# TravisWheelerLab/sufr

Hardware: AMD Instinct MI355X
Metric: suffixes sorted/sec (SA+LCP) (higher is better)
Workload: dtype u8 text / u32 indices / u64 packed keys; 1 GPU; syn_human 3.1 Gb stand-in for GRCh38, --dna --ignore-softmask -n 256 (BASELINE configs[3]); text_len=3100000001, num_suffixes=1500223556, parallelism=prefix-bucket shards x1, bits_per_char=3, radix_passes=5, digit_bits=15, levels=7, deep_records=58357696, placement_trials=3

## Files before the change

### profiles/micro/level2_pattern.hip

```cpp
#include <hip/hip_runtime.h>
#include <stdint.h>
#include <stdio.h>
#include <stdlib.h>
#include <vector>
#define CK(x) do { hipError_t e_ = (x); if (e_ != hipSuccess) { fprintf(stderr, "%s: %s\n", #x, hipGetErrorString(e_)); exit(1); } } while (0)
struct Rec12 { uint32_t a, b, c; };
struct Rec8 { uint32_t a, b; };

template <typename OUT>
__global__ void __launch_bounds__(512)
k_level2(const Rec12* __restrict__ in, OUT* __restrict__ out, uint32_t* __restrict__ cursor, uint32_t NB, uint32_t r, uint32_t SEG,
         uint32_t nseg)
{
    extern __shared__ uint32_t s_base[];
    const uint32_t g = blockIdx.x & 7u, w = blockIdx.x >> 3, R = gridDim.x >> 3;
    const uint32_t tile = NB * r, tps = SEG / tile;
    for (uint32_t seg = g; seg < nseg; seg += 8) {
        for (uint32_t t = w; t < tps; t += R) {
            __syncthreads();
            for (uint32_t d = threadIdx.x; d < NB; d += 512)
                s_base[d] = seg * SEG + d * (SEG / NB) + atomicAdd(&cursor[(size_t)seg * NB + d], r);
            __syncthreads();
            const Rec12* src = in + (size_t)seg * SEG + (size_t)t * tile;
            for (uint32_t j = threadIdx.x; j < tile; j += 512) {
                const Rec12 v = src[j];
                const uint32_t d = j / r, o = j - d * r;
                if constexpr (sizeof(OUT) == 12) out[(size_t)s_base[d] + o] = OUT{v.a, v.b, v.c};
                else out[(size_t)s_base[d] + o] = OUT{v.a ^ v.b, v.c};
            }
        }
    }
}

int main(int argc, char** argv)
{
    const uint32_t NB = argc > 1 ? (uint32_t)atoi(argv[1]) : 1400u;
    const uint32_t nseg = 1364;
    hipEvent_t e0, e1; CK(hipEventCreate(&e0)); CK(hipEventCreate(&e1));
    for (uint32_t r : {1u, 2u, 3u, 6u}) {
        const uint32_t tile = NB * r;
        const uint32_t SEG = (1100000u / tile) * tile;
        const uint64_t records = (uint64_t)SEG * nseg;
        Rec12* in; void* out; uint32_t* cursor;
        CK(hipMalloc(&in, records * 12)); CK(hipMalloc(&out, records * 12)); CK(hipMalloc(&cursor, (size_t)nseg * NB * 4));
        CK(hipMemset(in, 1, records * 12));
        for (int sz : {12, 8}) {
            float best = 1e9f;
            for (int rep = 0; rep < 3; rep++) {
                CK(hipMemset(cursor, 0, (size_t)nseg * NB * 4));
                CK(hipEventRecord(e0));
                if (sz == 12) hipLaunchKernelGGL(k_level2<Rec12>, dim3(1024), dim3(512), (size_t)NB * 4, 0, in, (Rec12*)out, cursor, NB, r, SEG, nseg);
                else hipLaunchKernelGGL(k_level2<Rec8>, dim3(1024), dim3(512), (size_t)NB * 4, 0, in, (Rec8*)out, cursor, NB, r, SEG, nseg);
                CK(hipEventRecord(e1)); CK(hipEventSynchronize(e1));
                float ms; CK(hipEventElapsedTime(&ms, e0, e1)); best = ms < best ? ms : best;
            }
            printf("sub-buckets %5u  run %u rec  out %2d B/rec : %7.2f ms  (%.3g records, %.1f GB read, %.1f GB written)\n", NB, r, sz, best,
                   (double)records, records * 12.0 / 1e9, records * (double)sz / 1e9);
        }
        CK(hipFree(in)); CK(hipFree(out)); CK(hipFree(cursor));
    }
    return 0;
}
```

### sufr_amd/csrc/sufr_launch.inc

```

#include <math.h>
#include <stdio.h>
#include <stdlib.h>
#include <string.h>

#include <chrono>
#include <memory>
#include <string>
#include <thread>
#include <vector>

#include "../../include/sufr_hip.h"

namespace sufr {

#define HIP_TRY(call)                                                                        \
    do {                                                                                     \
        hipError_t e__ = (call);                                                             \
        if (e__ != hipSuccess) {                                                             \
            set_error(std::string(#call) + ": " + hipGetErrorString(e__));                   \
            return SUFR_HIP_E_HIP;                                                           \
        }                                                                                    \
    } while (0)

// ... 23 lines not shown
    std::string err;
    uint64_t resident_text_len = 0;
    uint32_t stitch_weight = 0;
    uint64_t stitch_cap = 0;
    DevBuf stitchoffs;
    StitchOrder stitch_order() const { StitchOrder so; so.offs = stitch_weight ? (const uint32_t*)stitchoffs.p : nullptr; so.weight = stitch_weight; so.cap = stitch_cap; return so; }
    bool debug = false;

    DevBuf text, bytehist, lut, table, bintot, binbase, scalars;
    DevBuf keyA, keyB, idxA, idxB;
    DevBuf recA, recB;
    DevBuf rankbuf, dposbuf, deferbuf, unresbuf, posbitsbuf, dblf[7], dblg[6];
    DevBuf headsA, headsB, sizes, starts, partials;
    DevBuf tilefirst, runends, tileany, nexttile, nextblk, depthA, depthB, period, remapbuf, flagsbuf, packedbuf, wmaskbuf, wcntbuf, recoff, runoff, wlflag, wlhead, wloff, candbuf, keepbuf, plancnt, fixbuf;
    DevBuf rg_misc, rg_blk, rg_blkoff, rg_rs, rg_rl, rg_E, rg_L, rg_V, rg_tab[2], rg_off[2], rg_long[2], rg_tmax[2], rg_hist, rg_depth;
    DevBuf cumbuf, dmapbuf, identbuf[16], grouptab, gcur, leafcnt, leafoff, leafbase, leafcur, bigflag, bigoff;
    DevBuf rawtab, presbuf, rawtot, valsbuf, startbuf;
    DevBuf exc_pos, exc_byte, exc_sorted, exc_sa, exc_lcp, exc_bits, exc_blk, exc_off, exc_list, exc_list2, exc_pmin, exc_roff;
    std::unique_ptr<Pipeline> helper;
    bool overlap_chains = true;
    bool mql_fast_ok = true;
    bool exc_disable = false;
    bool no_exceptions = false;
    std::vector<uint32_t> rawtot_host, valshost;
    uint16_t h_lut[256];
    uint32_t h_seg0[2];
    DevBuf segst[2], segsz[2], tunits, upre, tdesc, wunits, wpre, wdesc, wslow;
    std::vector<uint8_t> dmaphost, identhost[16];
    std::vector<uint16_t> remaphost;
    std::vector<uint32_t> cumhost;
    int segcur = 0;
// ... 28 lines not shown
    uint32_t wide_shard_index = 0, wide_num_shards = 1;
    uint64_t wide_text_len = 0;
    uint64_t wide_orphans = 0;
    std::vector<uint32_t> opt_mask_offsets;
    hipEvent_t ev[16];
    bool have_events = false;

    static constexpr int LEAF_E = 8;
    int leaf_nt = 512;
    uint32_t LEAF_CAP = 4096;
    uint32_t LEAF_BIG = 4096;
    bool leaf_dna3 = false;
    uint32_t leaf_bmax = 256;
    int leaf_t1 = 12;
    int ms_e = 8;
    static constexpr int ms_nt = 512;

    void set_error(const std::string& s) { err = s; }

    static constexpr size_t PIN_CAP = (size_t)512 << 10;
    uint8_t* pin = nullptr;
    size_t pin_used = 0;
    struct PinItem { void* dst; size_t off, bytes; };
    std::vector<PinItem> pin_items;
    hipError_t d2h_at(void* dst, const void* src, size_t bytes)
    {
        if (!pin || pin_used + bytes > PIN_CAP) { copies_queued = true; return hipMemcpyAsync(dst, src, bytes, hipMemcpyDeviceToHost, stream); }
        const hipError_t e = hipMemcpyAsync(pin + pin_used, src, bytes, hipMemcpyDeviceToHost, stream);
        if (e == hipSuccess) { pin_items.push_back({dst, pin_used, bytes}); pin_used += (bytes + 63) & ~(size_t)63; copies_queued = true; }
        return e;
// ... 140 lines not shown
        if (const char* e = getenv("SUFR_PROBE_LEAF_BIG")) if (atoi(e) >= 64) LEAF_BIG = (uint32_t)atoi(e);
        if (LEAF_BIG > LEAF_CAP) LEAF_BIG = LEAF_CAP;
        if (const char* e = getenv("SUFR_PROBE_FINISH_OPTS")) finish_opts = (uint32_t)atoi(e) << 29;
        if (const char* e = getenv("SUFR_PROBE_DBL_SHARE")) dbl_min_share = (uint32_t)atoi(e);
        if (const char* e = getenv("SUFR_PROBE_P2MIN")) p2min_knob = atoi(e);
        key_carry = !getenv("SUFR_PROBE_NO_KEY_CARRY");
        run_groups = !getenv("SUFR_PROBE_NO_RUN_GROUPS");
        mask_lcp_from_keys = !getenv("SUFR_PROBE_MASK_LCP_TEXT");
        if (const char* e = getenv("SUFR_PROBE_MASK_DIGIT_BITS")) { int v = atoi(e); if (v >= 4 && v <= 12) mask_digit_bits = v; }
        if (const char* e = getenv("SUFR_PROBE_GROUP_SORT")) group_sort = atoi(e) != 0;
        if (const char* e = getenv("SUFR_PROBE_GIANT")) if (atoi(e) >= (int)GS_CAP) gs_giant_knob = (uint32_t)atoi(e);
        if (const char* e = getenv("SUFR_PROBE_KEY_CHARS")) key_chars_knob = atoi(e);
        if (const char* e = getenv("SUFR_PROBE_BMAX")) if (atoi(e) >= 1) leaf_bmax = (uint32_t)atoi(e);
        if (const char* e = getenv("SUFR_PROBE_LEAF_ABL")) leaf_bmax |= (uint32_t)atoi(e) << 24;
        if (const char* e = getenv("SUFR_PROBE_MS_E")) if (atoi(e) == 4 || atoi(e) == 6 || atoi(e) == 8) ms_e = atoi(e);
        if (const char* e = getenv("SUFR_PROBE_T1")) if (atoi(e) >= 11 && atoi(e) <= 13) leaf_t1 = atoi(e);
        if (leaf_nt == 512 && leaf_t1 == 13) leaf_t1 = 12;
        if (leaf_nt == 1024 && leaf_t1 == 11) leaf_t1 = 12;
#endif
        if (text_wgs > 16384u) text_wgs = 16384u;
        if (pairs_wgs > 16384u) pairs_wgs = 16384u;
    }

    void release(DevBuf& b) { if (b.p) (void)hipFree(b.p); b.p = nullptr; b.cap = 0; }

    void destroy()
    {
        if (helper) { helper->destroy(); helper.reset(); }
        (void)hipSetDevice(device);
        DevBuf* all[] = {&text, &bytehist, &lut, &table, &bintot, &binbase, &scalars, &keyA, &keyB, &idxA,
                         &idxB, &recA, &recB, &headsA, &headsB, &sizes, &starts, &partials, &sa32, &lcp32,
                         &tilefirst, &runends, &tileany, &nexttile, &nextblk, &depthA, &depthB, &period, &remapbuf, &flagsbuf, &packedbuf, &wmaskbuf, &wcntbuf, &recoff, &runoff, &wlflag, &wlhead, &wloff, &candbuf, &keepbuf, &plancnt, &fixbuf,
                         &rg_misc, &rg_blk, &rg_blkoff, &rg_rs, &rg_rl, &rg_E, &rg_L, &rg_V, &rg_tab[0], &rg_tab[1], &rg_off[0], &rg_off[1], &rg_long[0], &rg_long[1], &rg_tmax[0], &rg_tmax[1], &rg_hist, &rg_depth,
                         &exc_pos, &exc_byte, &exc_sorted, &exc_sa, &exc_lcp, &exc_bits, &exc_blk, &exc_off, &exc_list, &exc_list2, &exc_pmin, &exc_roff,
                         &cumbuf, &dmapbuf, &rawtab, &presbuf, &rawtot, &valsbuf, &startbuf, &grouptab, &gcur, &leafcnt, &leafoff, &leafbase, &leafcur, &bigflag, &bigoff,
                         &segst[0], &segst[1], &segsz[0], &segsz[1], &tunits, &upre, &tdesc, &wunits, &wpre, &wdesc, &wslow,
                         &optA, &optB, &optC, &optD, &optE, &stitchoffs, &wideoffs,
                         &gs_leafbase, &gs_pst, &gs_psz, &gs_wcnt, &gs_wpre, &gs_wdesc, &gs_flag, &gs_off, &gs_big, &gs_lg, &gs_lsz, &gs_loff};
        for (auto& b : identbuf) release(b);
        for (auto& b : dblf) release(b);
        for (auto& b : dblg) release(b);
        release(rankbuf); release(dposbuf); release(deferbuf); release(unresbuf); release(posbitsbuf);
        for (auto* b : all) release(*b);
        for (auto& l : lv) { release(l.keyA); release(l.keyB); release(l.idxA); release(l.idxB);
                             release(l.segA); release(l.segB); release(l.opos); }
        if (have_events) for (auto& e : ev) (void)hipEventDestroy(e);
        if (pin) { (void)hipHostFree(pin); pin = nullptr; }
        if (pub) { (void)hipHostFree(pub); pub = nullptr; pub_dev = nullptr; }
        if (own_stream && stream) (void)hipStreamDestroy(stream);
    }
// ... 514 lines not shown
        if ((rc = ensure(gs_loff, lcap * 4))) return rc;
        HIP_TRY(zero_later(gs_flag.p, cells * 4));
        HIP_TRY(zero_later(sc(SC_TMP0), 16));
        HIP_TRY(zero_later(sc(SC_GSLARGE), 16));
        HIP_TRY(zero_flush());
        hipLaunchKernelGGL(k_group_psegs, dim3((uint32_t)((cells + 255) / 256)), dim3(256), 0, stream, d_starts, L, m2, npseg,
                           (uint32_t*)gs_leafbase.p, (uint32_t*)gs_pst.p, (uint32_t*)gs_psz.p);
        if (maxsize > gs_giant) {
            hipLaunchKernelGGL(k_group_large, dim3((L + 255) / 256), dim3(256), 0, stream, d_sizes, L, gs_giant, sc(SC_GSLARGE),
                               (uint32_t*)gs_lg.p, (uint32_t*)gs_lsz.p);
            HIP_TRY(d2h_at(gp.large, sc(SC_GSLARGE), 16));
        }
        hipLaunchKernelGGL(k_pack_windows<false>, dim3((npseg + 3) / 4), dim3(256), 0, stream,
                           (const uint32_t*)gs_pst.p, (const uint32_t*)gs_psz.p, npseg, (const uint32_t*)gs_leafbase.p,
                           GS_PS, (uint32_t)GS_CAP, (uint32_t)GS_CAP, (uint32_t*)gs_wcnt.p, (const uint32_t*)nullptr,
                           (uint4*)nullptr, (uint32_t*)gs_flag.p);
        if ((rc = scan_u32((const uint32_t*)gs_wcnt.p, npseg, (uint32_t*)gs_wpre.p, sc(SC_TMP1)))) return rc;
        hipLaunchKernelGGL(k_pack_windows<true>, dim3((npseg + 3) / 4), dim3(256), 0, stream,
                           (const uint32_t*)gs_pst.p, (const uint32_t*)gs_psz.p, npseg, (const uint32_t*)gs_leafbase.p,
                           GS_PS, (uint32_t)GS_CAP, (uint32_t)GS_CAP, (uint32_t*)nullptr, (const uint32_t*)gs_wpre.p,
                           (uint4*)gs_wdesc.p, (uint32_t*)nullptr);
        if (maxsize > GS_CAP) {
            if ((rc = scan_u32((const uint32_t*)gs_flag.p, (uint32_t)cells, (uint32_t*)gs_off.p, sc(SC_GSBIG)))) return rc;
            hipLaunchKernelGGL(k_group_biglist, dim3((L + 255) / 256), dim3(256), 0, stream, (const uint32_t*)gs_flag.p,
                               (const uint32_t*)gs_off.p, L, (uint32_t*)gs_big.p);
        }
        HIP_TRY(hipGetLastError());
        return 0;
    }

    int group_sort_run(const GroupPlan& gp, uint64_t* k1, uint32_t* i1, const uint32_t* s1, uint64_t* k2, uint32_t* i2,
                       const uint32_t* d_starts, const uint32_t* d_sizes, uint32_t L, uint32_t m2, uint32_t maxsize,
                       int sort_bits, LevelArrays& C, bool& done)
    {
        int rc;
        (void)L;
// ... 587 lines not shown
        dm.rowbase = (const uint16_t*)((const uint8_t*)buf.p + (size_t)rows * 8);
        dm.rows = rows; dm.raw_mask = raw_bins - 1u; dm.nbins = dense; dm.dbits = dbits;
        return 0;
    }

    int identity_digit_map(int w, DigitMap& dm)
    {
        std::vector<uint32_t> all(1u << w, 1u);
        return upload_digit_map(all, w, identbuf[w], identhost[w], dm, nullptr);
    }

    static constexpr uint64_t SHARD_MIN_MQL = 8;
    static constexpr size_t PART_LDS_MAX = 160u * 1024u;
    static size_t msd_map_bytes_host(uint32_t rows) { return (size_t)rows * 8 + (((size_t)rows * 2 + 15) & ~(size_t)15); }

    int leaf_stage(const Rec* rsrc, Rec* rdst, uint32_t nseg, uint64_t m, const DigitMap& dm, const CharModel& cc,
                   const FinishOut& fo, int hibit, uint32_t& nbig, uint64_t& mbig, uint64_t& maxbig)
    {
        int rc;
        const uint32_t NB = dm.nbins;
        const uint64_t wub64 = 2 * (m / LEAF_CAP) + nseg + m / ((uint64_t)LEAF_BIG + 1) + 2;
        const uint64_t cells = (uint64_t)nseg * NB;
        if (wub64 >= (1ull << 31) || cells >= (1ull << 31)) { set_error("internal error: segment table too large"); return SUFR_HIP_E_HIP; }
        const uint32_t wub = (uint32_t)wub64;
        if ((rc = ensure(wunits, (size_t)nseg * 4))) return rc;
        if ((rc = ensure(wpre, (size_t)nseg * 4))) return rc;
        if ((rc = ensure(wdesc, (size_t)wub * 16))) return rc;
        if ((rc = ensure(bigflag, cells * 4))) return rc;
        if ((rc = ensure(bigoff, cells * 4))) return rc;
        if ((rc = ensure(wslow, (size_t)wub * 4))) return rc;
        HIP_TRY(zero_later(bigflag.p, cells * 4));
        HIP_TRY(zero_later(sc(SC_MBIG), 16));
        HIP_TRY(zero_later(wslow.p, (size_t)wub * 4));
        HIP_TRY(zero_flush());
        hipLaunchKernelGGL(k_pack_windows<false>, dim3((nseg + 3) / 4), dim3(256), 0, stream,
                           (const uint32_t*)segst[segcur].p, (const uint32_t*)segsz[segcur].p, nseg,
                           (const uint32_t*)leafbase.p, NB, (uint32_t)LEAF_CAP, (uint32_t)LEAF_BIG, (uint32_t*)wunits.p,
                           (const uint32_t*)nullptr, (uint4*)nullptr, (uint32_t*)bigflag.p);
        if ((rc = scan_u32((const uint32_t*)wunits.p, nseg, (uint32_t*)wpre.p, sc(SC_WTOTAL)))) return rc;
        hipLaunchKernelGGL(k_pack_windows<true>, dim3((nseg + 3) / 4), dim3(256), 0, stream,
                           (const uint32_t*)segst[segcur].p, (const uint32_t*)segsz[segcur].p, nseg,
                           (const uint32_t*)leafbase.p, NB, (uint32_t)LEAF_CAP, (uint32_t)LEAF_BIG, (uint32_t*)nullptr,
                           (const uint32_t*)wpre.p, (uint4*)wdesc.p, (uint32_t*)nullptr);
        if ((rc = scan_u32((const uint32_t*)bigflag.p, (uint32_t)cells, (uint32_t*)bigoff.p, sc(SC_NBIG)))) return rc;
        const uint64_t bigcap = m / (LEAF_BIG + 1) + 1;
        if ((rc = ensure(segst[segcur ^ 1], bigcap * 4))) return rc;
        if ((rc = ensure(segsz[segcur ^ 1], bigcap * 4))) return rc;
        hipLaunchKernelGGL(k_compact_big, dim3((uint32_t)((cells + 255) / 256)), dim3(256), 0, stream,
                           (const uint32_t*)bigflag.p, (const uint32_t*)bigoff.p, (const uint32_t*)leafbase.p,
                           (const uint32_t*)segst[segcur].p, (const uint32_t*)segsz[segcur].p, nseg, NB,
                           (uint32_t*)segst[segcur ^ 1].p, (uint32_t*)segsz[segcur ^ 1].p, sc(SC_MBIG));
        unsigned long long two[3] = {0, 0, 0};
        {
            const uint32_t gmax = leaf_nt == 1024 ? 1024u : 2048u;
            const uint32_t grid = wub < gmax ? wub : gmax;
            const size_t lds = (size_t)LEAF_CAP * 12 + msd_map_bytes_host(dm.rows) + (leaf_dna3 ? 0 : (size_t)LEAF_CS_MAX * 8) +
                               128 + ((size_t)1 << leaf_t1) * 4;
#define SUFR_LEAF(NT_, T1_, D3_)                                                                                         \
            {                                                                                                            \
                HIP_TRY(hipFuncSetAttribute((const void*)k_leaf_sort<NT_, LEAF_E, T1_, D3_>,                            \
                                            hipFuncAttributeMaxDynamicSharedMemorySize, (int)lds));                     \
                hipLaunchKernelGGL((k_leaf_sort<NT_, LEAF_E, T1_, D3_>), dim3(grid), dim3(NT_), lds, stream, rsrc,      \
                                   rdst, (const uint4*)wdesc.p, (const unsigned long long*)sc(SC_WTOTAL),              \
                                   (uint32_t*)wslow.p, hibit, dm, cc, fo, leaf_bmax);                                   \
            }
#define SUFR_LEAF_D(NT_, T1_) { if (leaf_dna3) SUFR_LEAF(NT_, T1_, true) else SUFR_LEAF(NT_, T1_, false) }
            if (leaf_nt == 1024) { if (leaf_t1 == 13) SUFR_LEAF_D(1024, 13) else SUFR_LEAF_D(1024, 12) }
// ... 5 lines not shown
#define SUFR_LEAF_LSD(NT_)                                                                                               \
            {                                                                                                            \
                HIP_TRY(hipFuncSetAttribute((const void*)k_leaf_sort_lsd<NT_, LEAF_E>,                                  \
                                            hipFuncAttributeMaxDynamicSharedMemorySize, (int)lds2));                    \
                hipLaunchKernelGGL((k_leaf_sort_lsd<NT_, LEAF_E>), dim3(grid), dim3(NT_), lds2, stream, rsrc, rdst,     \
                                   (const uint4*)wdesc.p, (const unsigned long long*)sc(SC_WTOTAL),                    \
                                   (const uint32_t*)wslow.p, hibit, cc.lastbit, dm, fo);                               \
            }
            if (leaf_nt == 1024) SUFR_LEAF_LSD(1024) else SUFR_LEAF_LSD(512)
#undef SUFR_LEAF_LSD
            hipLaunchKernelGGL(k_advance_fix, dim3(1), dim3(64), 0, stream, (uint32_t*)sc(SC_NFIX),
                               (const unsigned long long*)sc(SC_WTOTAL), 0u);
        }
        HIP_TRY(hipGetLastError());
        HIP_TRY(d2h(two, sc(SC_NBIG), 24));
        HIP_TRY(sync_reads());
        nbig = (uint32_t)two[0];
        mbig = two[1];
        maxbig = two[2];
        return 0;
    }

    int plan_tiles(uint32_t nseg, uint64_t m, uint32_t G, uint32_t unit, uint32_t& SG, uint32_t& tub)
    {
        int rc;
        SG = (nseg + G - 1) / G;
        const uint32_t slots = G * SG;
        tub = (uint32_t)(m / unit + nseg);
        if ((rc = ensure(tunits, (size_t)slots * 4))) return rc;
        if ((rc = ensure(upre, (size_t)slots * 4))) return rc;
        if ((rc = ensure(tdesc, (size_t)tub * 16))) return rc;
        hipLaunchKernelGGL(k_seg_units, dim3((slots + 255) / 256), dim3(256), 0, stream, (const uint32_t*)segsz[segcur].p,
                           nseg, G, SG, unit, (uint32_t*)tunits.p);
        if ((rc = scan_u32((const uint32_t*)tunits.p, slots, (uint32_t*)upre.p, sc(SC_UTOTAL)))) return rc;
// ... 555 lines not shown
        {
            if ((rc = ensure(segst[0], 256))) return rc;
            if ((rc = ensure(segsz[0], 256))) return rc;
            segcur = 0;
            h_seg0[0] = 0u; h_seg0[1] = m0;
            HIP_TRY(hipMemcpyAsync(segst[0].p, &h_seg0[0], 4, hipMemcpyHostToDevice, stream));
            HIP_TRY(hipMemcpyAsync(segsz[0].p, &h_seg0[1], 4, hipMemcpyHostToDevice, stream));
            uint32_t nseg = 1;
            uint64_t m = s;
            int src = 0;
            int bits_done = mbits;
            DigitMap dl = dm;
            const int maxbits = mql_fast ? 64 : kp.K * kp.b;
            const int charbits = mql_fast ? mql_charbits : maxbits;
            uint32_t levels = 1;
            for (;;) {
                uint32_t nbig = 0; uint64_t mbig = 0, maxbig = 0;
                if ((rc = leaf_stage(xr[src], xr[1], nseg, m, dl, cc, fo, 64 - bits_done, nbig, mbig, maxbig)))
                    return rc;
                if (debug) fprintf(stderr, "[sufr_hip debug] msd level %u: segments=%u records=%llu bits=%d -> big leaves=%u records=%llu\n",
                                   levels, nseg, (unsigned long long)m, bits_done, nbig, (unsigned long long)mbig);
                if (!nbig) break;
                segcur ^= 1; nseg = nbig; m = mbig;
                if (levels == 1 && packed_path && !mql_fast) {
                    if ((rc = run_groups_extract(d_text, n, kp, xr[src], xr[1], (uint32_t)(mbits / kp.b), s, fo, nseg, m, maxbig))) return rc;
                    if (!nseg) break;
                }
                int w = 0;
                const bool in_chars = bits_done < charbits;
                const int digit_end = in_chars ? charbits : maxbits;
                bool char_digit = false;
                if (bits_done < digit_end) {
                    w = mbits;
                    if (bits_done + w > digit_end) w = digit_end - bits_done;
                    uint64_t budget = (1ull << 26) / nseg;
                    int wb = 0; while (wb < 12 && (2ull << wb) <= budget) wb++;
// ... 23 lines not shown
                const uint64_t cells = (uint64_t)nseg * NBn;
                if ((rc = ensure(leafcnt, cells * 4))) return rc;
                if ((rc = ensure(leafoff, cells * 4))) return rc;
                if ((rc = ensure(leafbase, cells * 4))) return rc;
                if ((rc = ensure(leafcur, cells * 4))) return rc;
                HIP_TRY(hipMemsetAsync(leafcnt.p, 0, cells * 4, stream));
                {
                    const size_t lds = msd_map_bytes_host(dn.rows) + (size_t)NBn * 4;
                    hipLaunchKernelGGL(k_msd_hist, dim3(2048), dim3(THREADS), lds, stream, (const Rec*)xr[src],
                                       (const uint4*)tdesc.p, (const unsigned long long*)sc(SC_UTOTAL), shift, dn,
                                       (uint32_t*)leafcnt.p);
                }
                if ((rc = scan_u32((const uint32_t*)leafcnt.p, (uint32_t)cells, (uint32_t*)leafoff.p))) return rc;
                hipLaunchKernelGGL(k_msd_leafbase, dim3((uint32_t)((cells + 255) / 256)), dim3(256), 0, stream,
                                   (const uint32_t*)leafoff.p, (const uint32_t*)segst[segcur].p, nseg, NBn,
                                   (uint32_t*)leafbase.p, (uint32_t*)leafcur.p);
                {
#define SUFR_MSD_SCATTER(NT_, E_)                                                                                        \
                    {                                                                                                    \
                        const size_t lds = (size_t)(NT_ * E_) * 14 + msd_map_bytes_host(dn.rows) +                      \
                                           (size_t)((NBn + 3u) & ~3u) * 4 + 128;                                        \
                        HIP_TRY(hipFuncSetAttribute((const void*)k_msd_scatter<NT_, E_>,                                \
                                                    hipFuncAttributeMaxDynamicSharedMemorySize, (int)lds));             \
                        hipLaunchKernelGGL((k_msd_scatter<NT_, E_>), dim3(ms_e == 8 ? 1024 : 2048), dim3(NT_), lds, stream, \
                                           (const Rec*)xr[src], (const uint4*)tdesc.p, (const uint32_t*)upre.p, G, SG,  \
                                           (const unsigned long long*)sc(SC_UTOTAL), shift, dn, (uint32_t*)leafcur.p,   \
                                           xr[src ^ 1]);                                                                \
                    }
                    if (ms_e == 4) SUFR_MSD_SCATTER(512, 4) else if (ms_e == 6) SUFR_MSD_SCATTER(512, 6) else SUFR_MSD_SCATTER(512, 8)
#undef SUFR_MSD_SCATTER
                }
                HIP_TRY(hipGetLastError());
                src ^= 1;
                dl = dn;
                levels++;
            }
            st.num_passes = levels;
        }
        HIP_TRY(hipEventRecord(ev[6], stream));
        hipLaunchKernelGGL(k_fix_window_lcp, dim3(1024), dim3(256), 0, stream, (const uint32_t*)fixbuf.p,
                           (const uint32_t*)sc(SC_NFIX), fixcap, (const Rec*)xr[1], d_lcp, kp.b, kp.K);
// ... 231 lines not shown
```

### sufr_amd/csrc/sufr_msd.inc

```

namespace sufr {

static constexpr uint32_t MSD_MAX_BINS = 4096;

struct DigitMap {
    const uint64_t* pres;
    const uint16_t* rowbase;
    uint32_t rows;
    uint32_t raw_mask;
    uint32_t nbins;
    int dbits;
};

struct LdsMap {
    const uint64_t* pres;
    const uint16_t* rowbase;
};

__device__ __forceinline__ size_t msd_map_bytes(uint32_t rows) { return (size_t)rows * 8 + (((size_t)rows * 2 + 15) & ~(size_t)15); }

template <int NT>
__device__ __forceinline__ LdsMap msd_load_map(const DigitMap& dm, uint8_t* area)
{
    uint64_t* sp = reinterpret_cast<uint64_t*>(area);
// ... 503 lines not shown
                if (__ballot(d == d0) == ~0ull) { if (lane_id() == 0) atomicAdd(&s_cnt[d0], 64u); }
                else atomicAdd(&s_cnt[d], 1u);
            }
        }
        for (; i < td.y; i += THREADS) {
            const uint2 q = load_key_nt(&kp[i]);
            const uint64_t k = ((uint64_t)q.y << 32) | q.x;
            atomicAdd(&s_cnt[dense_digit((uint32_t)(k >> shift) & dm.raw_mask, map)], 1u);
        }
    }
    if (seg != 0xffffffffu) flush(seg);
}

__global__ void __launch_bounds__(256)
k_msd_leafbase(const uint32_t* __restrict__ off, const uint32_t* __restrict__ seg_start, uint32_t nseg, uint32_t NB,
               uint32_t* __restrict__ leafbase, uint32_t* __restrict__ leafcur)
{
    const uint64_t i = (uint64_t)blockIdx.x * 256 + threadIdx.x;
    if (i >= (uint64_t)nseg * NB) return;
    const uint32_t k = (uint32_t)(i / NB);
    const uint32_t v = seg_start[k] + (off[i] - off[(size_t)k * NB]);
    leafbase[i] = v;
    leafcur[i] = v;
}

template <int NT, int E>
__global__ void __launch_bounds__(NT)
k_msd_scatter(const Rec* __restrict__ in, const uint4* __restrict__ tdesc, const uint32_t* __restrict__ upre,
              uint32_t G, uint32_t SG, const unsigned long long* __restrict__ utotal, int shift, DigitMap dm,
              uint32_t* __restrict__ leafcur, Rec* __restrict__ out)
{
    constexpr int TILEB = NT * E;
    extern __shared__ __align__(16) uint8_t smem[];
    const uint32_t NB = dm.nbins;
    const uint32_t NBa = (NB + 3u) & ~3u;
    uint64_t* s_key = reinterpret_cast<uint64_t*>(smem);
    const LdsMap map = msd_load_map<NT>(dm, smem + (size_t)TILEB * 8);
    uint32_t* s_idx = reinterpret_cast<uint32_t*>(smem + (size_t)TILEB * 8 + msd_map_bytes(dm.rows));
    uint32_t* s_cnt = s_idx + TILEB;
    uint32_t* s_misc = s_cnt + NBa;
    uint16_t* s_dig = reinterpret_cast<uint16_t*>(s_misc + 32);

    const uint32_t g = blockIdx.x % G, r = blockIdx.x / G, R = gridDim.x / G;
    const uint32_t lo = upre[(size_t)g * SG];
    const uint32_t hi = (g + 1 < G) ? upre[(size_t)(g + 1) * SG] : (uint32_t)*utotal;
    uint32_t nlo[E], nhi[E], nix[E];
    uint4 ntd = make_uint4(0u, 0u, 0u, 0u);
    auto fetch = [&](uint32_t t) {
        ntd = tdesc[t];
#pragma unroll
        for (int e = 0; e < E; e++) {
            const uint32_t j = (uint32_t)e * NT + threadIdx.x;
            nlo[e] = 0; nhi[e] = 0; nix[e] = 0;
            if (j < ntd.y) { const Rec rr = in[ntd.x + j]; nlo[e] = rr.klo; nhi[e] = rr.khi; nix[e] = rr.idx; }
        }
    };
    auto pin = [&]() {
#pragma unroll
        for (int e = 0; e < E; e++) asm volatile("" : "+v"(nlo[e]), "+v"(nhi[e]), "+v"(nix[e]));
    };
    if (lo + r < hi) { fetch(lo + r); pin(); }
    SUFR_STAMP_DECL(8)
    for (uint32_t t = lo + r; t < hi; t += R) {
        const uint4 td = ntd;
        __syncthreads();
        SUFR_STAMP(ph__, 0)
        for (uint32_t i = threadIdx.x; i < NB; i += NT) s_cnt[i] = 0;
        uint64_t key[E];
        uint32_t idx[E], dig[E], rank[E];
        uint32_t valid = 0;
#pragma unroll
        for (int e = 0; e < E; e++) {
            const uint32_t j = (uint32_t)e * NT + threadIdx.x;
            key[e] = ((uint64_t)nhi[e] << 32) | nlo[e]; idx[e] = nix[e];
            if (j < td.y) valid |= 1u << e;
        }
#pragma unroll
        for (int e = 0; e < E; e++) dig[e] = dense_digit((uint32_t)(key[e] >> shift) & dm.raw_mask, map);
        __syncthreads();
        SUFR_STAMP(ph__, 1)
#pragma unroll
        for (int e = 0; e < E; e++) {
            const bool v = valid & (1u << e);
            const uint64_t vm = __ballot(v);
            const uint32_t d0 = (uint32_t)__builtin_amdgcn_readfirstlane((int)dig[e]);
            if (vm == ~0ull && __ballot(dig[e] == d0) == ~0ull) {
                uint32_t b = 0;
                if (lane_id() == 0) b = atomicAdd(&s_cnt[d0], 64u);
                rank[e] = (uint32_t)__builtin_amdgcn_readfirstlane((int)b) + lane_id();
            } else {
                rank[e] = v ? atomicAdd(&s_cnt[dig[e]], 1u) : 0u;
            }
        }
        __syncthreads();
        SUFR_STAMP(ph__, 2)
        MsdClaim<NT> cl;
        msd_claim_begin<NT>(s_cnt, NB, leafcur + (size_t)td.z * NB, s_misc, s_misc + 24, cl);
        SUFR_STAMP(ph__, 3)
        const bool more = t + R < hi;
        if (more) fetch(t + R);
#pragma unroll
        for (int e = 0; e < E; e++) {
            if (valid & (1u << e)) {
                const uint32_t pos = s_cnt[dig[e]] + rank[e];
                s_key[pos] = key[e];
                s_idx[pos] = idx[e];
                s_dig[pos] = (uint16_t)dig[e];
            }
        }
        SUFR_STAMP(ph__, 4)
        msd_claim_end<NT>(s_cnt, NB, cl);
        SUFR_STAMP(ph__, 5)
        if (more) pin();
        SUFR_STAMP(ph__, 6)
        for (uint32_t j = threadIdx.x; j < td.y; j += NT) {
            const uint32_t o = j + s_cnt[s_dig[j]];
            out[o] = make_rec(s_key[j], s_idx[j]);
        }
        SUFR_STAMP(ph__, 7)
    }
    SUFR_STAMP_FLUSH(1, 8)
}

__global__ void __launch_bounds__(256)
k_copy_tiles(const Rec* __restrict__ in, const uint4* __restrict__ tdesc,
             const unsigned long long* __restrict__ utotal, Rec* __restrict__ out)
{
    const uint32_t T = (uint32_t)*utotal;
    for (uint32_t t = blockIdx.x; t < T; t += gridDim.x) {
        const uint4 td = tdesc[t];
        for (uint32_t j = threadIdx.x; j < td.y; j += 256) out[td.x + j] = in[td.x + j];
    }
}

template <bool EMIT>
__global__ void __launch_bounds__(256)
k_pack_windows(const uint32_t* __restrict__ seg_start, const uint32_t* __restrict__ seg_size, uint32_t nseg,
               const uint32_t* __restrict__ leafbase, uint32_t NB, uint32_t CAP, uint32_t BIG,
               uint32_t* __restrict__ wcount, const uint32_t* __restrict__ wpre, uint4* __restrict__ wdesc,
               uint32_t* __restrict__ bigflag)
{
    const uint32_t k = blockIdx.x * 4 + (threadIdx.x >> 6);
    if (k >= nseg) return;
    const uint32_t ln = lane_id();
    const uint32_t* lb = leafbase + (size_t)k * NB;
    const uint32_t s0 = seg_start[k], s1 = s0 + seg_size[k];
    (void)s0;
    bool open = false;
    uint32_t wpos = 0, wleaf = 0, nw = 0;
    const uint32_t wbase = EMIT ? wpre[k] : 0u;
    auto close = [&](uint32_t endpos, uint32_t endleaf) {
        if (endpos > wpos) {
            if (EMIT && ln == 0u) wdesc[wbase + nw] = make_uint4(wpos, endpos - wpos, wleaf, endleaf - wleaf);
            nw++;
        }
        open = false;
    };
    for (uint32_t c = 0; c < NB; c += 64) {
        const uint32_t d = c + ln;
        const bool valid = d < NB;
        const uint32_t b = valid ? lb[d] : s1;
        const uint32_t e = (d + 1 < NB) ? lb[d + 1] : s1;
        const bool big = valid && e - b > BIG;
        if (!EMIT && big) bigflag[(size_t)k * NB + d] = 1u;
        const uint32_t nv = min(64u, NB - c);
        uint32_t cur = 0;
        while (cur < nv) {
            if (!open) {
                const uint64_t nb = __ballot(valid && !big) & (~0ull << cur);
                if (!nb) break;
                cur = (uint32_t)__builtin_ctzll(nb);
                wpos = (uint32_t)__builtin_amdgcn_readlane((int)b, (int)cur);
                wleaf = c + cur;
                open = true;
            }
            const uint64_t stop = __ballot(valid && (big || e - wpos > CAP)) & (~0ull << cur);
            if (!stop) break;
            cur = (uint32_t)__builtin_ctzll(stop);
            close((uint32_t)__builtin_amdgcn_readlane((int)b, (int)cur), c + cur);
        }
    }
    if (open) close(s1, NB);
    if (!EMIT && ln == 0u) wcount[k] = nw;
}

__global__ void __launch_bounds__(256)
k_compact_big(const uint32_t* __restrict__ bigflag, const uint32_t* __restrict__ bigoff,
              const uint32_t* __restrict__ leafbase, const uint32_t* __restrict__ seg_start,
              const uint32_t* __restrict__ seg_size, uint32_t nseg, uint32_t NB,
              uint32_t* __restrict__ new_start, uint32_t* __restrict__ new_size,
              unsigned long long* __restrict__ big_records )
{
    const uint64_t i = (uint64_t)blockIdx.x * 256 + threadIdx.x;
    if (i >= (uint64_t)nseg * NB || !bigflag[i]) return;
    const uint32_t k = (uint32_t)(i / NB), d = (uint32_t)(i % NB);
    const uint32_t a = leafbase[i];
    const uint32_t b = d + 1 < NB ? leafbase[i + 1] : seg_start[k] + seg_size[k];
    new_start[bigoff[i]] = a;
// ... 768 lines not shown
```

Measured before the change: 29.37 billion suffixes/s.

## Scatter MSD records by leaf-window targets instead of per-sub-bucket digits

The level planning (window packing) now runs before the MSD scatter. It emits a per-segment map from sub-bucket digit to target, where a target is a packed leaf window or a big leaf, and it initialises the target cursors. The scatter kernel loads that map into LDS, counts and claims per target rather than per digit, and packs rank and target into one register. This shrinks the count/claim loop and the number of global atomic cursors, and it raises the launch bound to four blocks per CU. In exchange the plan work moves earlier, there is an extra LDS row load per segment, and the records inside a window are no longer split by digit at scatter time.

```diff
diff --git a/profiles/micro/level2_pattern.hip b/profiles/micro/level2_pattern.hip
--- a/profiles/micro/level2_pattern.hip
+++ b/profiles/micro/level2_pattern.hip
@@ -35,27 +35,34 @@
 int main(int argc, char** argv)
 {
     const uint32_t NB = argc > 1 ? (uint32_t)atoi(argv[1]) : 1400u;
-    const uint32_t nseg = 1364;
+    const uint32_t seg_arg = argc > 2 ? (uint32_t)atoi(argv[2]) : 1100000u;
+    std::vector<uint32_t> runs;
+    for (int a = 3; a < argc; a++) if (atoi(argv[a]) > 0) runs.push_back((uint32_t)atoi(argv[a]));
+    if (runs.empty()) runs = {1u, 2u, 3u, 6u};
+    if (NB == 0 || seg_arg == 0) { fprintf(stderr, "usage: level2_pattern [NB [SEG [r ...]]]\n"); return 2; }
     hipEvent_t e0, e1; CK(hipEventCreate(&e0)); CK(hipEventCreate(&e1));
-    for (uint32_t r : {1u, 2u, 3u, 6u}) {
+    for (uint32_t r : runs) {
         const uint32_t tile = NB * r;
-        const uint32_t SEG = (1100000u / tile) * tile;
+        if (tile > seg_arg) { fprintf(stderr, "a tile of %u records does not fit a segment of %u\n", tile, seg_arg); return 2; }
+        const uint32_t SEG = (seg_arg / tile) * tile;
+        const uint32_t nseg = (uint32_t)(1364ull * 1100000ull / SEG);
         const uint64_t records = (uint64_t)SEG * nseg;
         Rec12* in; void* out; uint32_t* cursor;
         CK(hipMalloc(&in, records * 12)); CK(hipMalloc(&out, records * 12)); CK(hipMalloc(&cursor, (size_t)nseg * NB * 4));
         CK(hipMemset(in, 1, records * 12));
         for (int sz : {12, 8}) {
-            float best = 1e9f;
-            for (int rep = 0; rep < 3; rep++) {
+            float best = 1e9f, all[5];
+            for (int rep = 0; rep < 5; rep++) {
                 CK(hipMemset(cursor, 0, (size_t)nseg * NB * 4));
                 CK(hipEventRecord(e0));
                 if (sz == 12) hipLaunchKernelGGL(k_level2<Rec12>, dim3(1024), dim3(512), (size_t)NB * 4, 0, in, (Rec12*)out, cursor, NB, r, SEG, nseg);
                 else hipLaunchKernelGGL(k_level2<Rec8>, dim3(1024), dim3(512), (size_t)NB * 4, 0, in, (Rec8*)out, cursor, NB, r, SEG, nseg);
                 CK(hipEventRecord(e1)); CK(hipEventSynchronize(e1));
-                float ms; CK(hipEventElapsedTime(&ms, e0, e1)); best = ms < best ? ms : best;
+                float ms; CK(hipEventElapsedTime(&ms, e0, e1)); best = ms < best ? ms : best; all[rep] = ms;
             }
-            printf("sub-buckets %5u  run %u rec  out %2d B/rec : %7.2f ms  (%.3g records, %.1f GB read, %.1f GB written)\n", NB, r, sz, best,
-                   (double)records, records * 12.0 / 1e9, records * (double)sz / 1e9);
+            printf("sub-buckets %5u  run %u rec  out %2d B/rec : %7.2f ms  (%.3g records, %.1f GB read, %.1f GB written; segments of %u; "
+                   "runs %.2f %.2f %.2f %.2f %.2f)\n", NB, r, sz, best, (double)records, records * 12.0 / 1e9, records * (double)sz / 1e9, SEG,
+                   all[0], all[1], all[2], all[3], all[4]);
         }
         CK(hipFree(in)); CK(hipFree(out)); CK(hipFree(cursor));
     }
diff --git a/sufr_amd/csrc/sufr_launch.inc b/sufr_amd/csrc/sufr_launch.inc
--- a/sufr_amd/csrc/sufr_launch.inc
+++ b/sufr_amd/csrc/sufr_launch.inc
@@ -61,7 +61,7 @@
     DevBuf headsA, headsB, sizes, starts, partials;
     DevBuf tilefirst, runends, tileany, nexttile, nextblk, depthA, depthB, period, remapbuf, flagsbuf, packedbuf, wmaskbuf, wcntbuf, recoff, runoff, wlflag, wlhead, wloff, candbuf, keepbuf, plancnt, fixbuf;
     DevBuf rg_misc, rg_blk, rg_blkoff, rg_rs, rg_rl, rg_E, rg_L, rg_V, rg_tab[2], rg_off[2], rg_long[2], rg_tmax[2], rg_hist, rg_depth;
-    DevBuf cumbuf, dmapbuf, identbuf[16], grouptab, gcur, leafcnt, leafoff, leafbase, leafcur, bigflag, bigoff;
+    DevBuf cumbuf, dmapbuf, identbuf[16], grouptab, gcur, leafcnt, leafoff, leafbase, leafcur, leaftgt, ntgt, bigflag, bigoff;
     DevBuf rawtab, presbuf, rawtot, valsbuf, startbuf;
     DevBuf exc_pos, exc_byte, exc_sorted, exc_sa, exc_lcp, exc_bits, exc_blk, exc_off, exc_list, exc_list2, exc_pmin, exc_roff;
     std::unique_ptr<Pipeline> helper;
@@ -120,6 +120,7 @@
     uint32_t leaf_bmax = 256;
     int leaf_t1 = 12;
     int ms_e = 8;
+    bool ms_leaf_targets = false;
     static constexpr int ms_nt = 512;
 
     void set_error(const std::string& s) { err = s; }
@@ -290,6 +291,7 @@
         if (const char* e = getenv("SUFR_PROBE_BMAX")) if (atoi(e) >= 1) leaf_bmax = (uint32_t)atoi(e);
         if (const char* e = getenv("SUFR_PROBE_LEAF_ABL")) leaf_bmax |= (uint32_t)atoi(e) << 24;
         if (const char* e = getenv("SUFR_PROBE_MS_E")) if (atoi(e) == 4 || atoi(e) == 6 || atoi(e) == 8) ms_e = atoi(e);
+        ms_leaf_targets = getenv("SUFR_PROBE_MS_LEAF_TARGETS") && atoi(getenv("SUFR_PROBE_MS_LEAF_TARGETS"));
         if (const char* e = getenv("SUFR_PROBE_T1")) if (atoi(e) >= 11 && atoi(e) <= 13) leaf_t1 = atoi(e);
         if (leaf_nt == 512 && leaf_t1 == 13) leaf_t1 = 12;
         if (leaf_nt == 1024 && leaf_t1 == 11) leaf_t1 = 12;
@@ -309,7 +311,7 @@
                          &tilefirst, &runends, &tileany, &nexttile, &nextblk, &depthA, &depthB, &period, &remapbuf, &flagsbuf, &packedbuf, &wmaskbuf, &wcntbuf, &recoff, &runoff, &wlflag, &wlhead, &wloff, &candbuf, &keepbuf, &plancnt, &fixbuf,
                          &rg_misc, &rg_blk, &rg_blkoff, &rg_rs, &rg_rl, &rg_E, &rg_L, &rg_V, &rg_tab[0], &rg_tab[1], &rg_off[0], &rg_off[1], &rg_long[0], &rg_long[1], &rg_tmax[0], &rg_tmax[1], &rg_hist, &rg_depth,
                          &exc_pos, &exc_byte, &exc_sorted, &exc_sa, &exc_lcp, &exc_bits, &exc_blk, &exc_off, &exc_list, &exc_list2, &exc_pmin, &exc_roff,
-                         &cumbuf, &dmapbuf, &rawtab, &presbuf, &rawtot, &valsbuf, &startbuf, &grouptab, &gcur, &leafcnt, &leafoff, &leafbase, &leafcur, &bigflag, &bigoff,
+                         &cumbuf, &dmapbuf, &rawtab, &presbuf, &rawtot, &valsbuf, &startbuf, &grouptab, &gcur, &leafcnt, &leafoff, &leafbase, &leafcur, &leaftgt, &ntgt, &bigflag, &bigoff,
                          &segst[0], &segst[1], &segsz[0], &segsz[1], &tunits, &upre, &tdesc, &wunits, &wpre, &wdesc, &wslow,
                          &optA, &optB, &optC, &optD, &optE, &stitchoffs, &wideoffs,
                          &gs_leafbase, &gs_pst, &gs_psz, &gs_wcnt, &gs_wpre, &gs_wdesc, &gs_flag, &gs_off, &gs_big, &gs_lg, &gs_lsz, &gs_loff};
@@ -854,12 +856,12 @@
         hipLaunchKernelGGL(k_pack_windows<false>, dim3((npseg + 3) / 4), dim3(256), 0, stream,
                            (const uint32_t*)gs_pst.p, (const uint32_t*)gs_psz.p, npseg, (const uint32_t*)gs_leafbase.p,
                            GS_PS, (uint32_t)GS_CAP, (uint32_t)GS_CAP, (uint32_t*)gs_wcnt.p, (const uint32_t*)nullptr,
-                           (uint4*)nullptr, (uint32_t*)gs_flag.p);
+                           (uint4*)nullptr, (uint32_t*)gs_flag.p, (uint16_t*)nullptr, (uint32_t*)nullptr, (uint32_t*)nullptr);
         if ((rc = scan_u32((const uint32_t*)gs_wcnt.p, npseg, (uint32_t*)gs_wpre.p, sc(SC_TMP1)))) return rc;
         hipLaunchKernelGGL(k_pack_windows<true>, dim3((npseg + 3) / 4), dim3(256), 0, stream,
                            (const uint32_t*)gs_pst.p, (const uint32_t*)gs_psz.p, npseg, (const uint32_t*)gs_leafbase.p,
                            GS_PS, (uint32_t)GS_CAP, (uint32_t)GS_CAP, (uint32_t*)nullptr, (const uint32_t*)gs_wpre.p,
-                           (uint4*)gs_wdesc.p, (uint32_t*)nullptr);
+                           (uint4*)gs_wdesc.p, (uint32_t*)nullptr, (uint16_t*)nullptr, (uint32_t*)nullptr, (uint32_t*)nullptr);
         if (maxsize > GS_CAP) {
             if ((rc = scan_u32((const uint32_t*)gs_flag.p, (uint32_t)cells, (uint32_t*)gs_off.p, sc(SC_GSBIG)))) return rc;
             hipLaunchKernelGGL(k_group_biglist, dim3((L + 255) / 256), dim3(256), 0, stream, (const uint32_t*)gs_flag.p,
@@ -1477,15 +1479,17 @@
     static constexpr size_t PART_LDS_MAX = 160u * 1024u;
     static size_t msd_map_bytes_host(uint32_t rows) { return (size_t)rows * 8 + (((size_t)rows * 2 + 15) & ~(size_t)15); }
 
-    int leaf_stage(const Rec* rsrc, Rec* rdst, uint32_t nseg, uint64_t m, const DigitMap& dm, const CharModel& cc,
-                   const FinishOut& fo, int hibit, uint32_t& nbig, uint64_t& mbig, uint64_t& maxbig)
+    int leaf_plan(uint32_t nseg, uint64_t m, uint32_t NB, bool targets, uint32_t& wub)
     {
         int rc;
-        const uint32_t NB = dm.nbins;
         const uint64_t wub64 = 2 * (m / LEAF_CAP) + nseg + m / ((uint64_t)LEAF_BIG + 1) + 2;
         const uint64_t cells = (uint64_t)nseg * NB;
         if (wub64 >= (1ull << 31) || cells >= (1ull << 31)) { set_error("internal error: segment table too large"); return SUFR_HIP_E_HIP; }
-        const uint32_t wub = (uint32_t)wub64;
+        wub = (uint32_t)wub64;
+        if (targets) {
+            if ((rc = ensure(leaftgt, (size_t)nseg * msd_tgt_stride(NB) * 2))) return rc;
+            if ((rc = ensure(ntgt, (size_t)nseg * 4))) return rc;
+        }
         if ((rc = ensure(wunits, (size_t)nseg * 4))) return rc;
         if ((rc = ensure(wpre, (size_t)nseg * 4))) return rc;
         if ((rc = ensure(wdesc, (size_t)wub * 16))) return rc;
@@ -1499,12 +1503,20 @@
         hipLaunchKernelGGL(k_pack_windows<false>, dim3((nseg + 3) / 4), dim3(256), 0, stream,
                            (const uint32_t*)segst[segcur].p, (const uint32_t*)segsz[segcur].p, nseg,
                            (const uint32_t*)leafbase.p, NB, (uint32_t)LEAF_CAP, (uint32_t)LEAF_BIG, (uint32_t*)wunits.p,
-                           (const uint32_t*)nullptr, (uint4*)nullptr, (uint32_t*)bigflag.p);
+                           (const uint32_t*)nullptr, (uint4*)nullptr, (uint32_t*)bigflag.p, (uint16_t*)nullptr,
+                           (uint32_t*)nullptr, (uint32_t*)nullptr);
         if ((rc = scan_u32((const uint32_t*)wunits.p, nseg, (uint32_t*)wpre.p, sc(SC_WTOTAL)))) return rc;
         hipLaunchKernelGGL(k_pack_windows<true>, dim3((nseg + 3) / 4), dim3(256), 0, stream,
                            (const uint32_t*)segst[segcur].p, (const uint32_t*)segsz[segcur].p, nseg,
                            (const uint32_t*)leafbase.p, NB, (uint32_t)LEAF_CAP, (uint32_t)LEAF_BIG, (uint32_t*)nullptr,
-                           (const uint32_t*)wpre.p, (uint4*)wdesc.p, (uint32_t*)nullptr);
+                           (const uint32_t*)wpre.p, (uint4*)wdesc.p, (uint32_t*)nullptr,
+                           targets ? (uint16_t*)leaftgt.p : (uint16_t*)nullptr, targets ? (uint32_t*)leafcur.p : (uint32_t*)nullptr,
+                           targets ? (uint32_t*)ntgt.p : (uint32_t*)nullptr);
+#ifdef SUFR_HIP_PROBES
+        if (targets && ms_leaf_targets)
+            hipLaunchKernelGGL(k_msd_leaf_targets, dim3((uint32_t)((cells + 255) / 256)), dim3(256), 0, stream,
+                               (const uint32_t*)leafbase.p, nseg, NB, (uint16_t*)leaftgt.p, (uint32_t*)leafcur.p, (uint32_t*)ntgt.p);
+#endif
         if ((rc = scan_u32((const uint32_t*)bigflag.p, (uint32_t)cells, (uint32_t*)bigoff.p, sc(SC_NBIG)))) return rc;
         const uint64_t bigcap = m / (LEAF_BIG + 1) + 1;
         if ((rc = ensure(segst[segcur ^ 1], bigcap * 4))) return rc;
@@ -1513,7 +1525,14 @@
                            (const uint32_t*)bigflag.p, (const uint32_t*)bigoff.p, (const uint32_t*)leafbase.p,
                            (const uint32_t*)segst[segcur].p, (const uint32_t*)segsz[segcur].p, nseg, NB,
                            (uint32_t*)segst[segcur ^ 1].p, (uint32_t*)segsz[segcur ^ 1].p, sc(SC_MBIG));
-        unsigned long long two[3] = {0, 0, 0};
+        HIP_TRY(hipGetLastError());
+        return 0;
+    }
+
+    int leaf_sort(const Rec* rsrc, Rec* rdst, uint32_t wub, const DigitMap& dm, const CharModel& cc, const FinishOut& fo, int hibit,
+                  uint32_t& nbig, uint64_t& mbig, uint64_t& maxbig, uint64_t& nwindows)
+    {
+        unsigned long long two[3] = {0, 0, 0}, wtot = 0;
         {
             const uint32_t gmax = leaf_nt == 1024 ? 1024u : 2048u;
             const uint32_t grid = wub < gmax ? wub : gmax;
@@ -1549,10 +1568,12 @@
         }
         HIP_TRY(hipGetLastError());
         HIP_TRY(d2h(two, sc(SC_NBIG), 24));
+        if (debug) HIP_TRY(d2h(&wtot, sc(SC_WTOTAL), 8));
         HIP_TRY(sync_reads());
         nbig = (uint32_t)two[0];
         mbig = two[1];
         maxbig = two[2];
+        nwindows = wtot;
         return 0;
     }
 
@@ -2138,12 +2159,14 @@
             const int maxbits = mql_fast ? 64 : kp.K * kp.b;
             const int charbits = mql_fast ? mql_charbits : maxbits;
             uint32_t levels = 1;
+            uint32_t wub = 0;
+            if ((rc = leaf_plan(nseg, m, dl.nbins, false, wub))) return rc;
             for (;;) {
-                uint32_t nbig = 0; uint64_t mbig = 0, maxbig = 0;
-                if ((rc = leaf_stage(xr[src], xr[1], nseg, m, dl, cc, fo, 64 - bits_done, nbig, mbig, maxbig)))
+                uint32_t nbig = 0; uint64_t mbig = 0, maxbig = 0, nwindows = 0;
+                if ((rc = leaf_sort(xr[src], xr[1], wub, dl, cc, fo, 64 - bits_done, nbig, mbig, maxbig, nwindows)))
                     return rc;
-                if (debug) fprintf(stderr, "[sufr_hip debug] msd level %u: segments=%u records=%llu bits=%d -> big leaves=%u records=%llu\n",
-                                   levels, nseg, (unsigned long long)m, bits_done, nbig, (unsigned long long)mbig);
+                if (debug) fprintf(stderr, "[sufr_hip debug] msd level %u: segments=%u records=%llu bits=%d -> windows=%llu big leaves=%u records=%llu\n",
+                                   levels, nseg, (unsigned long long)m, bits_done, (unsigned long long)nwindows, nbig, (unsigned long long)mbig);
                 if (!nbig) break;
                 segcur ^= 1; nseg = nbig; m = mbig;
                 if (levels == 1 && packed_path && !mql_fast) {
@@ -2197,17 +2220,20 @@
                 if ((rc = scan_u32((const uint32_t*)leafcnt.p, (uint32_t)cells, (uint32_t*)leafoff.p))) return rc;
                 hipLaunchKernelGGL(k_msd_leafbase, dim3((uint32_t)((cells + 255) / 256)), dim3(256), 0, stream,
                                    (const uint32_t*)leafoff.p, (const uint32_t*)segst[segcur].p, nseg, NBn,
-                                   (uint32_t*)leafbase.p, (uint32_t*)leafcur.p);
+                                   (uint32_t*)leafbase.p);
+                if ((rc = leaf_plan(nseg, m, NBn, true, wub))) return rc;
                 {
 #define SUFR_MSD_SCATTER(NT_, E_)                                                                                        \
                     {                                                                                                    \
-                        const size_t lds = (size_t)(NT_ * E_) * 14 + msd_map_bytes_host(dn.rows) +                      \
-                                           (size_t)((NBn + 3u) & ~3u) * 4 + 128;                                        \
+                        const size_t lds = (size_t)(NT_ * E_) * 12 + msd_map_bytes_host(dn.rows) +                      \
+                                           (size_t)((NBn + 3u) & ~3u) * 4 + 128 +                                       \
+                                           (size_t)std::max<uint32_t>(NT_ * E_, msd_tgt_stride(NBn)) * 2;               \
                         HIP_TRY(hipFuncSetAttribute((const void*)k_msd_scatter<NT_, E_>,                                \
                                                     hipFuncAttributeMaxDynamicSharedMemorySize, (int)lds));             \
                         hipLaunchKernelGGL((k_msd_scatter<NT_, E_>), dim3(ms_e == 8 ? 1024 : 2048), dim3(NT_), lds, stream, \
                                            (const Rec*)xr[src], (const uint4*)tdesc.p, (const uint32_t*)upre.p, G, SG,  \
-                                           (const unsigned long long*)sc(SC_UTOTAL), shift, dn, (uint32_t*)leafcur.p,   \
+                                           (const unsigned long long*)sc(SC_UTOTAL), shift, dn,                         \
+                                           (const uint16_t*)leaftgt.p, (const uint32_t*)ntgt.p, (uint32_t*)leafcur.p,   \
                                            xr[src ^ 1]);                                                                \
                     }
                     if (ms_e == 4) SUFR_MSD_SCATTER(512, 4) else if (ms_e == 6) SUFR_MSD_SCATTER(512, 6) else SUFR_MSD_SCATTER(512, 8)
diff --git a/sufr_amd/csrc/sufr_msd.inc b/sufr_amd/csrc/sufr_msd.inc
--- a/sufr_amd/csrc/sufr_msd.inc
+++ b/sufr_amd/csrc/sufr_msd.inc
@@ -541,40 +541,66 @@
 
 __global__ void __launch_bounds__(256)
 k_msd_leafbase(const uint32_t* __restrict__ off, const uint32_t* __restrict__ seg_start, uint32_t nseg, uint32_t NB,
-               uint32_t* __restrict__ leafbase, uint32_t* __restrict__ leafcur)
+               uint32_t* __restrict__ leafbase)
 {
     const uint64_t i = (uint64_t)blockIdx.x * 256 + threadIdx.x;
     if (i >= (uint64_t)nseg * NB) return;
     const uint32_t k = (uint32_t)(i / NB);
-    const uint32_t v = seg_start[k] + (off[i] - off[(size_t)k * NB]);
-    leafbase[i] = v;
-    leafcur[i] = v;
-}
+    leafbase[i] = seg_start[k] + (off[i] - off[(size_t)k * NB]);
+}
+
+__host__ __device__ __forceinline__ uint32_t msd_tgt_stride(uint32_t NB) { return (NB + 7u) & ~7u; }
+
+#ifdef SUFR_HIP_PROBES
+__global__ void __launch_bounds__(256)
+k_msd_leaf_targets(const uint32_t* __restrict__ leafbase, uint32_t nseg, uint32_t NB, uint16_t* __restrict__ leaftgt,
+                   uint32_t* __restrict__ leafcur, uint32_t* __restrict__ ntgt)
+{
+    const uint64_t i = (uint64_t)blockIdx.x * 256 + threadIdx.x;
+    if (i >= (uint64_t)nseg * NB) return;
+    const uint32_t k = (uint32_t)(i / NB), d = (uint32_t)(i % NB);
+    leaftgt[(size_t)k * msd_tgt_stride(NB) + d] = (uint16_t)d;
+    leafcur[i] = leafbase[i];
+    if (d == 0) ntgt[k] = NB;
+}
+#endif
 
 template <int NT, int E>
-__global__ void __launch_bounds__(NT)
+__global__ void __launch_bounds__(NT, 4)
 k_msd_scatter(const Rec* __restrict__ in, const uint4* __restrict__ tdesc, const uint32_t* __restrict__ upre,
               uint32_t G, uint32_t SG, const unsigned long long* __restrict__ utotal, int shift, DigitMap dm,
+              const uint16_t* __restrict__ leaftgt, const uint32_t* __restrict__ ntgt,
               uint32_t* __restrict__ leafcur, Rec* __restrict__ out)
 {
     constexpr int TILEB = NT * E;
+    static_assert(NT * 8 >= (int)MSD_MAX_BINS, "a thread carries eight entries of the target row");
+    static_assert(TILEB <= 65536 && MSD_MAX_BINS <= 65536, "target and rank share a register");
     extern __shared__ __align__(16) uint8_t smem[];
     const uint32_t NB = dm.nbins;
     const uint32_t NBa = (NB + 3u) & ~3u;
+    const uint32_t NBs = msd_tgt_stride(NB);
     uint64_t* s_key = reinterpret_cast<uint64_t*>(smem);
     const LdsMap map = msd_load_map<NT>(dm, smem + (size_t)TILEB * 8);
     uint32_t* s_idx = reinterpret_cast<uint32_t*>(smem + (size_t)TILEB * 8 + msd_map_bytes(dm.rows));
     uint32_t* s_cnt = s_idx + TILEB;
     uint32_t* s_misc = s_cnt + NBa;
     uint16_t* s_dig = reinterpret_cast<uint16_t*>(s_misc + 32);
+    uint16_t* s_row = s_dig;
 
     const uint32_t g = blockIdx.x % G, r = blockIdx.x / G, R = gridDim.x / G;
     const uint32_t lo = upre[(size_t)g * SG];
     const uint32_t hi = (g + 1 < G) ? upre[(size_t)(g + 1) * SG] : (uint32_t)*utotal;
     uint32_t nlo[E], nhi[E], nix[E];
     uint4 ntd = make_uint4(0u, 0u, 0u, 0u);
+    uint4 nrow = make_uint4(0u, 0u, 0u, 0u);
+    uint32_t rowseg = 0xffffffffu, nT = 0;
     auto fetch = [&](uint32_t t) {
         ntd = tdesc[t];
+        if (ntd.z != rowseg) {
+            rowseg = ntd.z;
+            nT = ntgt[rowseg];
+            if (threadIdx.x * 8u < NBs) nrow = reinterpret_cast<const uint4*>(leaftgt + (size_t)rowseg * NBs)[threadIdx.x];
+        }
 #pragma unroll
         for (int e = 0; e < E; e++) {
             const uint32_t j = (uint32_t)e * NT + threadIdx.x;
@@ -585,16 +611,22 @@
     auto pin = [&]() {
 #pragma unroll
         for (int e = 0; e < E; e++) asm volatile("" : "+v"(nlo[e]), "+v"(nhi[e]), "+v"(nix[e]));
+        asm volatile("" : "+v"(nrow.x), "+v"(nrow.y), "+v"(nrow.z), "+v"(nrow.w));
     };
     if (lo + r < hi) { fetch(lo + r); pin(); }
     SUFR_STAMP_DECL(8)
     for (uint32_t t = lo + r; t < hi; t += R) {
         const uint4 td = ntd;
+        const uint32_t T = nT;
         __syncthreads();
         SUFR_STAMP(ph__, 0)
-        for (uint32_t i = threadIdx.x; i < NB; i += NT) s_cnt[i] = 0;
+        for (uint32_t i = threadIdx.x; i < T; i += NT) s_cnt[i] = 0;
+        if (threadIdx.x * 8u < NBs) {
+            reinterpret_cast<uint2*>(s_row)[2u * threadIdx.x] = make_uint2(nrow.x, nrow.y);
+            reinterpret_cast<uint2*>(s_row)[2u * threadIdx.x + 1u] = make_uint2(nrow.z, nrow.w);
+        }
         uint64_t key[E];
-        uint32_t idx[E], dig[E], rank[E];
+        uint32_t idx[E], tr[E];
         uint32_t valid = 0;
 #pragma unroll
         for (int e = 0; e < E; e++) {
@@ -603,40 +635,44 @@
             if (j < td.y) valid |= 1u << e;
         }
 #pragma unroll
-        for (int e = 0; e < E; e++) dig[e] = dense_digit((uint32_t)(key[e] >> shift) & dm.raw_mask, map);
+        for (int e = 0; e < E; e++) tr[e] = dense_digit((uint32_t)(key[e] >> shift) & dm.raw_mask, map);
         __syncthreads();
         SUFR_STAMP(ph__, 1)
+#pragma unroll
+        for (int e = 0; e < E; e++) tr[e] = (valid & (1u << e)) ? (uint32_t)s_row[tr[e]] : 0u;
 #pragma unroll
         for (int e = 0; e < E; e++) {
             const bool v = valid & (1u << e);
             const uint64_t vm = __ballot(v);
-            const uint32_t d0 = (uint32_t)__builtin_amdgcn_readfirstlane((int)dig[e]);
-            if (vm == ~0ull && __ballot(dig[e] == d0) == ~0ull) {
+            const uint32_t d0 = (uint32_t)__builtin_amdgcn_readfirstlane((int)tr[e]);
+            uint32_t rank;
+            if (vm == ~0ull && __ballot(tr[e] == d0) == ~0ull) {
                 uint32_t b = 0;
                 if (lane_id() == 0) b = atomicAdd(&s_cnt[d0], 64u);
-                rank[e] = (uint32_t)__builtin_amdgcn_readfirstlane((int)b) + lane_id();
+                rank = (uint32_t)__builtin_amdgcn_readfirstlane((int)b) + lane_id();
             } else {
-                rank[e] = v ? atomicAdd(&s_cnt[dig[e]], 1u) : 0u;
-            }
+                rank = v ? atomicAdd(&s_cnt[tr[e]], 1u) : 0u;
+            }
+            tr[e] |= rank << 16;
         }
         __syncthreads();
         SUFR_STAMP(ph__, 2)
         MsdClaim<NT> cl;
-        msd_claim_begin<NT>(s_cnt, NB, leafcur + (size_t)td.z * NB, s_misc, s_misc + 24, cl);
+        msd_claim_begin<NT>(s_cnt, T, leafcur + (size_t)td.z * NB, s_misc, s_misc + 24, cl);
         SUFR_STAMP(ph__, 3)
         const bool more = t + R < hi;
         if (more) fetch(t + R);
 #pragma unroll
         for (int e = 0; e < E; e++) {
             if (valid & (1u << e)) {
-                const uint32_t pos = s_cnt[dig[e]] + rank[e];
+                const uint32_t pos = s_cnt[tr[e] & 0xffffu] + (tr[e] >> 16);
                 s_key[pos] = key[e];
                 s_idx[pos] = idx[e];
-                s_dig[pos] = (uint16_t)dig[e];
+                s_dig[pos] = (uint16_t)tr[e];
             }
         }
         SUFR_STAMP(ph__, 4)
-        msd_claim_end<NT>(s_cnt, NB, cl);
+        msd_claim_end<NT>(s_cnt, T, cl);
         SUFR_STAMP(ph__, 5)
         if (more) pin();
         SUFR_STAMP(ph__, 6)
@@ -665,7 +701,8 @@
 k_pack_windows(const uint32_t* __restrict__ seg_start, const uint32_t* __restrict__ seg_size, uint32_t nseg,
                const uint32_t* __restrict__ leafbase, uint32_t NB, uint32_t CAP, uint32_t BIG,
                uint32_t* __restrict__ wcount, const uint32_t* __restrict__ wpre, uint4* __restrict__ wdesc,
-               uint32_t* __restrict__ bigflag)
+               uint32_t* __restrict__ bigflag, uint16_t* __restrict__ leaftgt,
+               uint32_t* __restrict__ tgtcur, uint32_t* __restrict__ ntgt)
 {
     const uint32_t k = blockIdx.x * 4 + (threadIdx.x >> 6);
     if (k >= nseg) return;
@@ -676,6 +713,8 @@
     bool open = false;
     uint32_t wpos = 0, wleaf = 0, nw = 0;
     const uint32_t wbase = EMIT ? wpre[k] : 0u;
+    const bool targets = EMIT && leaftgt != nullptr;
+    uint32_t nt = 0;
     auto close = [&](uint32_t endpos, uint32_t endleaf) {
         if (endpos > wpos) {
             if (EMIT && ln == 0u) wdesc[wbase + nw] = make_uint4(wpos, endpos - wpos, wleaf, endleaf - wleaf);
@@ -692,11 +731,13 @@
         if (!EMIT && big) bigflag[(size_t)k * NB + d] = 1u;
         const uint32_t nv = min(64u, NB - c);
         uint32_t cur = 0;
+        uint64_t opened = 0;
         while (cur < nv) {
             if (!open) {
                 const uint64_t nb = __ballot(valid && !big) & (~0ull << cur);
                 if (!nb) break;
                 cur = (uint32_t)__builtin_ctzll(nb);
+                opened |= 1ull << cur;
                 wpos = (uint32_t)__builtin_amdgcn_readlane((int)b, (int)cur);
                 wleaf = c + cur;
                 open = true;
@@ -706,9 +747,19 @@
             cur = (uint32_t)__builtin_ctzll(stop);
             close((uint32_t)__builtin_amdgcn_readlane((int)b, (int)cur), c + cur);
         }
+        if (targets) {
+            const uint64_t first = opened | __ballot(big);
+            if (valid) {
+                const uint32_t t = nt + (uint32_t)__popcll(first & (~0ull >> (63u - ln))) - 1u;
+                leaftgt[(size_t)k * msd_tgt_stride(NB) + d] = (uint16_t)t;
+                if ((first >> ln) & 1ull) tgtcur[(size_t)k * NB + t] = b;
+            }
+            nt += (uint32_t)__popcll(first);
+        }
     }
     if (open) close(s1, NB);
     if (!EMIT && ln == 0u) wcount[k] = nw;
+    if (targets && ln == 0u) ntgt[k] = nt;
 }
 
 __global__ void __launch_bounds__(256)
```

Measured after the change: 29.71 billion suffixes/s (median of 6 runs). 1.2% higher.
